# lightec-xyz/bls-verify-gadget

Hardware: AMD Instinct MI355X
Metric: BLS-verify witness instances/sec (full pairing circuit) (higher is better)
Workload: dtype u32 (381-bit Montgomery integers mod the BLS12-381 prime as 12 x 32-bit limbs in memory, products on 14 x 28-bit limbs with 64-bit columns; SHA-256 words)

## Files before the change

__graft_entry__.py:

```python
import importlib
import os
import subprocess
import sys

ROOT = os.path.dirname(os.path.abspath(__file__))
if ROOT not in sys.path:
    sys.path.insert(0, ROOT)


def build():
    pkg = importlib.import_module("bls-verify-gadget_amd")
    pkg.build(force=False)
    subprocess.check_call(["make", "-s", "-C", os.path.join(ROOT, "oracle")])
    subprocess.check_call(["make", "-s", "-C", os.path.join(ROOT, "tests", "hostsim")])
    subprocess.check_call(["make", "-s", "-C", os.path.join(ROOT, "tests", "msg_input")])
    subprocess.check_call(["make", "-s", "-C", os.path.join(ROOT, "tests", "agg_inputs")])
    subprocess.check_call(["make", "-s", "-C", os.path.join(ROOT, "tests", "c_caller")])
    subprocess.check_call(["make", "-s", "-C", os.path.join(ROOT, "tests", "cpp_caller")])
    pkg.lib()
    for s in pkg.EXPORTED_SYMBOLS:
        getattr(pkg.lib(), s)


def smoke():
    import numpy as np
    import torch

    from tests import oracle_lib, synth

    pkg = importlib.import_module("bls-verify-gadget_amd")
    o = oracle_lib.load()
# ... 21 lines not shown
```

bls-verify-gadget_amd/build.py:

```python
import concurrent.futures
import hashlib
import os
import subprocess
import sys

HERE = os.path.dirname(os.path.abspath(__file__))
CSRC = os.path.join(HERE, "csrc")
OUT = os.path.join(HERE, "libblsw.so")
OBJ = os.path.join(HERE, "build_obj")
SOURCES = ["engine.hip", "k_agg_io.hip", "k_bench.hip", "k_cofactor.hip", "k_cofv.hip", "k_g1.hip", "k_g2.hip", "k_map.hip", "k_miller_par.hip", "k_msg.hip", "k_pairing_lane.hip", "k_prepare.hip", "k_r1cs.hip", "k_sha.hip",
           "k_sign.hip", "k_stream.hip", "k_team.hip", "k_values.hip"]
HOST_SOURCES = ["r1cs.cpp"]
HEADERS = sorted(f for f in os.listdir(CSRC) if f.endswith((".hpp", ".h")))
_SHORT_W2 = "the short chains: +4 % on the 20-step job at two waves, neutral in the steady state (profiles/r03_ab_chain_builds.txt)"
CHAIN_UNITS = {
    "k_sha.hip": ("W2", ("inl",), _SHORT_W2),
    "k_g1.hip": ("W2", ("inl",), _SHORT_W2),
    "k_g2.hip": ("OUTLINE", ("inl", "q"), "inlined it takes the whole file and the expansion starves; at two waves it spills 590 registers into its hot loop "
                 "(profiles/r03_ab_chain_builds.txt)"),
    "k_map.hip": ("W2", ("inl", "q"), _SHORT_W2),
    "k_cofactor.hip": ("OUTLINE", ("inl",), "inlined it takes the whole file and the expansion starves; at two waves it spills 2 400 registers into its hot loop "
                       "(profiles/r03_ab_chain_builds.txt)"),
    "k_prepare.hip": ("W2", ("inl", "q"), _SHORT_W2),
    "k_cofv.hip": ("FULL", ("q",), "the serial phases and the join: at two waves the join spills 2 000 registers into its additions"),
}
# ... 136 lines not shown
```

bls-verify-gadget_amd/csrc/chains.hpp:

```cpp
#pragma once
#include "curve.hpp"
#include "tower.hpp"

namespace blsw {

BLSW_HD bool bit_of(const uint32_t* words, int i) { return (words[i >> 5] >> (i & 31)) & 1; }

BLSW_FN bool fp_is_eq_pre_w(Emitter& e, const Fp& diff, const Fp& diff_inv) {
    bool ne = !fp_is_zero(diff);
    e.put_bool(ne);
    e.put(ne ? diff_inv : fp_one());
    return !ne;
}

struct G1ChainOut {
    Fp ax, ay;
};
BLSW_FN Proj<OpsFp> chain_g1_alloc_only(Emitter e_alloc, const Fp& pkx, const Fp& pky) {
    constexpr uint32_t H1[4] = BLSW_H1_WORDS;
    constexpr uint32_t H1INV[8] = BLSW_H1INV_WORDS;
    bool inf = fp_is_zero(pkx) && fp_is_zero(pky);
    Jac1 acc = {pkx, pky, fp_one()};
#pragma unroll 1
    for (int i = BLSW_H1INV_NBITS - 2; i >= 0; i--) {
        acc = jac1_dbl(acc);
        if (bit_of(H1INV, i)) acc = jac1_add_mixed(acc, pkx, pky);
    }
    Fp zi = fp_inv(acc.z);
    Fp zi2 = fp_sqr(zi);
    Fp px = fp_mul(acc.x, zi2), py = fp_mul(acc.y, fp_mul(zi2, zi));
    Proj<OpsFp> ge;
    ge.x = inf ? fp_zero() : px;
    ge.y = inf ? fp_one() : py;
    ge.z = inf ? fp_zero() : fp_one();
    e_alloc.put(ge.x);
    e_alloc.put(ge.y);
    e_alloc.put(ge.z);
    return proj_mul_bits_be_w<OpsFp>(e_alloc, ge, H1, BLSW_H1_NBITS);
}
BLSW_FN G1ChainOut chain_g1_post(Emitter e_notzero, Emitter e_prep, const Proj<OpsFp>& pk) {
    Fp nz = fp_neg(pk.z);
    Fp nzi = fp_inv(nz);
    bool x_eq = fp_is_eq_pre_w(e_notzero, fp_zero(), fp_zero());
    bool y_eq = fp_is_eq_pre_w(e_notzero, nz, nzi);
    bool coords_eq = x_eq && y_eq;
    e_notzero.put_bool(coords_eq);
    bool z_is_zero = fp_is_eq_pre_w(e_notzero, nz, nzi);
    e_notzero.put_bool(!z_is_zero && !coords_eq);
    bool infinity = fp_is_eq_pre_w(e_prep, nz, nzi);
    Fp z_inv = fp_neg(nzi);
    e_prep.put(z_inv);
    Fp nzx = fp_mul_w(e_prep, pk.x, z_inv);
    Fp nzy = fp_mul_w(e_prep, pk.y, z_inv);
// ... 32 lines not shown
    Fp2 l0 = fp2_mul_w(e, ge.x, ge.z);
    Fp2 r0 = fp2_mul_w(e, ge.x, ge.z);
    bool x_eq = fp2_is_eq_w(e, l0, r0);
    Fp2 l1 = fp2_mul_w(e, ge.y, ge.z);
    Fp2 r1 = fp2_mul_w(e, ge.y, ge.z);
    bool y_eq = fp2_is_eq_w(e, l1, r1);
    bool coords_eq = x_eq && y_eq;
    e.put_bool(coords_eq);
    bool za = fp2_is_zero_w(e, ge.z);
    bool zb = fp2_is_zero_w(e, ge.z);
    bool both_zero = za && zb;
    e.put_bool(both_zero);
    e.put_bool(both_zero || coords_eq);
}

BLSW_FN void chain_g2_alloc(Emitter e, const Fp2& sx, const Fp2& sy) {
    constexpr uint32_t RM1[8] = BLSW_RM1_WORDS;
    bool inf = fp2_is_zero(sx) && fp2_is_zero(sy);
    Proj<OpsFp2> ge;
    ge.x = inf ? fp2_zero() : sx;
    ge.y = inf ? fp2_one() : sy;
    ge.z = inf ? fp2_zero() : fp2_one();
    e.put(ge.x.c0);
    e.put(ge.x.c1);
    e.put(ge.y.c0);
    e.put(ge.y.c1);
    e.put(ge.z.c0);
    e.put(ge.z.c1);
    (void)proj_mul_bits_be_w<OpsFp2>(e, ge, RM1, BLSW_RM1_NBITS);
    chain_g2_alloc_tail(e, ge);
}

BLSW_FN Fp2 sswu_pow_c1_w(Emitter& e, const Fp2& v) {
    constexpr uint32_t C1[24] = BLSW_SSWU_C1_WORDS;
    Fp2 r = v;
#pragma unroll 1
    for (int i = BLSW_SSWU_C1_NBITS - 4; i >= 0; i--) {
        r = fp2_sqr_w(e, r);
        if (bit_of(C1, i)) r = fp2_mul_w(e, r, v);
    }
    return r;
}
BLSW_FN bool sswu_sgn0_w(Emitter& e, const Fp2& v) {
    bool sign_0 = fp_to_bits_le_w(e, v.c0);
// ... 381 lines not shown
```

bls-verify-gadget_amd/csrc/curve.hpp:

```cpp
#pragma once
#include "constants.hpp"
#include "gadgets.hpp"

namespace blsw {

struct OpsFp {
    typedef Fp F;
    static BLSW_HD F add(const F& a, const F& b) { return fp_add(a, b); }
    static BLSW_HD F sub(const F& a, const F& b) { return fp_sub(a, b); }
    static BLSW_HD F dbl(const F& a) { return fp_dbl(a); }
    static BLSW_HD F neg(const F& a) { return fp_neg(a); }
    static BLSW_HD F mul_w(Emitter& e, const F& a, const F& b) { return fp_mul_w(e, a, b); }
    static BLSW_HD F sqr_w(Emitter& e, const F& a) { return fp_mul_w(e, a, a); }
    static BLSW_HD F mul3b(const F& a) {
        F a4 = fp_dbl(fp_dbl(a));
        return fp_add(fp_dbl(a4), a4);
    }
    static BLSW_HD F one() { return fp_one(); }
    static BLSW_HD F zero() { return fp_zero(); }
    static BLSW_HD F k3b() { return K_G1_3B(); }
};
struct OpsFp2 {
    typedef Fp2 F;
    static BLSW_HD F add(const F& a, const F& b) { return fp2_add(a, b); }
// ... 70 lines not shown
    F m3 = O::mul_w(e, xx3, bxz3);
    F y = O::add(m2, m3);
    F m4 = O::mul_w(e, yy_p, yz_pairs);
    F m5 = O::mul_w(e, xy_pairs, xx3);
    F z = O::add(m4, m5);
    return {x, y, z};
}
template <class O>
BLSW_FN Proj<O> proj_double_w(Emitter& e, const Proj<O>& p) {
    return proj_double_inl<O>(e, p);
}
template <class O, int ZMODE>
BLSW_FN Proj<O> proj_add_w(Emitter& e, const Proj<O>& a, const Proj<O>& b) {
    return proj_add_inl<O, ZMODE>(e, a, b);
}
template <class O>
BLSW_FN Proj<O> proj_mul_bits_be_w(Emitter& e, const Proj<O>& ge, const uint32_t* words, int nbits) {
    Proj<O> result = ge;
#pragma unroll 1
    for (int i = nbits - 2; i >= 0; i--) {
        result = proj_double_inl<O>(e, result);
        if ((words[i >> 5] >> (i & 31)) & 1) result = proj_add_inl<O, 0>(e, result, ge);
    }
    return result;
}

struct Aff2 {
    Fp2 x, y;
};
BLSW_FN Aff2 nz_double_w(Emitter& e, const Aff2& p) {
    Fp2 x1_sqr = fp2_sqr_w(e, p.x);
    Fp2 num = fp2_add(fp2_dbl(x1_sqr), x1_sqr);
    Fp2 den = fp2_dbl(p.y);
    Fp2 lambda = fp2_div_w(e, num, den);
    Fp2 l2 = fp2_sqr_w(e, lambda);
// ... 95 lines not shown
```

bls-verify-gadget_amd/csrc/engine.hip:

```cpp
#include <cstdio>
#include <cstdlib>
#include <deque>
#include <map>
#include <vector>
#include "kcommon.hpp"
#include "agg_input.hpp"

using namespace blsw;

namespace {

inline int hip_ok(hipError_t e, const char* what) {
    if (e != hipSuccess) {
        fprintf(stderr, "[blsw] %s: %s\n", what, hipGetErrorString(e));
        return BLSW_ERR_HIP;
    }
    return BLSW_OK;
}

struct DeviceGuard {
    int prev = -1;
    bool switched = false;
    explicit DeviceGuard(int dev) {
        if (dev < 0) return;
// ... 101 lines not shown
    }
    if (e->sha) hipStreamDestroy(e->sha);
    if (e->expand) hipStreamDestroy(e->expand);
    if (e->place) hipStreamDestroy(e->place);
    if (e->lat) hipStreamDestroy(e->lat);
    if (e->ev_exp) {
        for (int i = 0; i < 2 * BLSW_MAX_TIMED; i++)
            if (e->ev_exp[i]) hipEventDestroy(e->ev_exp[i]);
        delete[] e->ev_exp;
    }
    for (int i = 0; i < BLSW_MAX_CONSUMED; i++)
        if (e->consumed_ev[i]) hipEventDestroy(e->consumed_ev[i]);
    delete e;
}

static void launch_place(blsw_engine* e, hipStream_t st, const Fp* staging, const Fp* pair, uint32_t split_row, uint64_t first, uint64_t* out, uint64_t out_stride) {
    const uint32_t rows = e->L.n_witness - e->L.sha_bits;
    const unsigned chunks = (rows * 3 + 256 * BLSW_PLACE_ITERS - 1) / (256 * BLSW_PLACE_ITERS);
    dim3 grid2(8 * ((chunks + 7) / 8) * (unsigned)e->n);
    hipLaunchKernelGGL(k_place_field, grid2, dim3(256), 0, st, staging, pair, first, e->L.off_expand, e->L.sha_bits, rows, split_row, out, out_stride, (uint32_t)e->n,
                       e->L.off_sig_alloc, e->modes.g2_team ? e->L.off_pk_not_zero - e->L.off_sig_alloc : 0u, e->LS.off_sig_alloc);
}
static void launch_place_multi(blsw_engine* e, hipStream_t st, const Workspace& ws, const Fp* pair_tiles, uint64_t first_pair, const Fp* inst_tiles, uint64_t first_inst,
                               uint32_t inst_tile_w, const Fp* rows, uint64_t* out, uint64_t out_stride) {
    const blsw_layout_t& L = e->L;
    const blsw_layout_t& S = e->LS;
    const uint32_t K = L.n_pairs, n = (uint32_t)e->n;
    PlaceRuns pr = {};
    pr.n_runs = 6;
    const uint32_t src[7] = {S.off_msg, S.off_pk_alloc, S.off_pk_not_zero, S.off_map0, S.off_prep_h, S.off_prep_pk, ws.rows_p};
    const uint32_t dst[6] = {L.off_msg, L.off_pk_alloc, L.off_pk_not_zero, L.off_map0, L.off_prep_h, L.off_prep_pk};
    const uint32_t str[6] = {L.stride_msg, L.stride_pk_alloc, L.stride_pk_not_zero, L.stride_hash, L.stride_prep_h, L.stride_prep_pk};
    for (int r = 0; r < 7; r++) pr.src_row[r] = src[r];
    for (int r = 0; r < 6; r++) pr.dst_off[r] = dst[r], pr.dst_stride[r] = str[r];
    auto blocks = [](uint32_t rows_, uint32_t n_y) {
        const unsigned chunks = (rows_ * 3 + 256 * BLSW_PLACE_ITERS - 1) / (256 * BLSW_PLACE_ITERS);
// ... 72 lines not shown
    hipEventRecord(b.ev_x[s], e->expand);
    hipStreamWaitEvent(e->place, b.ev_chains, 0);
    hipStreamWaitEvent(e->place, b.ev_x[s], 0);
    if (d.compact) {
        char* dst = reinterpret_cast<char*>(d.compact);
        hipMemcpyAsync(dst + cf.off_staging, ws.staging + (uint64_t)s * (e->n * Kc / 64) * ws.rows_p * 64, cf.staging_bytes, hipMemcpyDeviceToDevice, e->place);
        if (cf.inst_bytes) {
            const uint64_t lane0 = (uint64_t)s * e->n;
            const Fp* src = ws.staging_inst + (lane0 >> 6) * (uint64_t)ws.rows_i * 64 + (lane0 & 63);
            if (cf.inst_tile_w == 64)
                hipMemcpyAsync(dst + cf.off_inst, src, cf.inst_bytes, hipMemcpyDeviceToDevice, e->place);
            else
                hipMemcpy2DAsync(dst + cf.off_inst, e->n * sizeof(Fp), src, 64 * sizeof(Fp), e->n * sizeof(Fp), ws.rows_i, hipMemcpyDeviceToDevice, e->place);
        }
        if (cf.pair_bytes) hipMemcpyAsync(dst + cf.off_pair, ws.pair + (uint64_t)s * e->n * ws.pair_rows, cf.pair_bytes, hipMemcpyDeviceToDevice, e->place);
    }
    if (d.out && e->staged) {
        if (e->L.n_pairs > 1)
            launch_place_multi(e, e->place, ws, ws.staging, (uint64_t)s * e->n * e->L.n_pairs, ws.staging_inst, (uint64_t)s * e->n, 64u,
                               ws.pair + (uint64_t)s * e->n * ws.pair_rows, d.out, d.out_stride);
        else
            launch_place(e, e->place, ws.staging, ws.pair, ws.split_row, (uint64_t)s * e->n, d.out, d.out_stride);
    }
    if (d.out && e->opt.output_form) launch_canonical(e, e->place, d.out, d.out_stride);
    hipEventRecord(b.ev_step[s], e->place);
}
static int pump(blsw_engine* e) {
    while (!e->jobs.empty()) {
        const Job j = e->jobs.front();
        GroupBuf& b = e->buf[j.buf];
        const StepDesc& d = b.h_desc[j.s];
        const void* ptr = tracked_output(e, d);
        int slot = -1;
        if (ptr) {
            slot = consumed_slot(e, ptr);
            if (slot < 0) return BLSW_ERR_ARG;
            if (e->held[slot]) break;
// ... 269 lines not shown
    o->pk_mode = 0;
    o->sig_mode = 0;
    o->msg_mode = 0;
    o->agg_inputs = 0;
    return BLSW_OK;
}

int blsw_engine_workspace_bytes_ex(uint64_t n, uint32_t msg_len, uint32_t max_steps, uint32_t n_buffers, const blsw_engine_options_t* options, uint64_t* bytes) {
    if (!bytes) return BLSW_ERR_ARG;
    if (int rc = check_options(n, msg_len, max_steps, n_buffers, options)) return rc;
    blsw_layout_t L;
    const uint32_t K = options->n_pairs > 1 ? options->n_pairs : 1;
    options_layout(msg_len, options, &L);
    const bool staged = max_steps > 1 || n_buffers > 1;
    uint64_t need = 0;
    const Modes all[3] = {{true, false}, {true, true}, {false, false}};
    const uint64_t small_steps = BLSW_LATENCY_MAX_LANES / (n * K) < max_steps ? BLSW_LATENCY_MAX_LANES / (n * K) : max_steps;
    for (const Modes& m : all) {
        uint64_t t = carve(nullptr, n * max_steps * K, L, staged, m, n * max_steps).total_bytes;
        need = t > need ? t : need;
        if (small_steps) {
            t = carve(nullptr, n * small_steps * K, L, staged, m, n * small_steps).total_bytes;
            need = t > need ? t : need;
        }
    }
    if (K > 1) need = align_up(need, 256) + miller_par_bytes(n * max_steps, K);
    *bytes = (uint64_t)n_buffers * align_up(need, 4096);
    return BLSW_OK;
}
int blsw_engine_workspace_bytes(uint64_t n, uint32_t msg_len, uint32_t max_steps, uint32_t n_buffers, uint64_t* bytes) {
    blsw_engine_options_t o;
// ... 23 lines not shown
        if (hipFuncGetAttributes(&fa, reinterpret_cast<const void*>(k_pairing)) == hipSuccess && fa.localSizeBytes) stack = fa.localSizeBytes;
        const uint64_t projected = stack * 64ull * (uint64_t)cus * 32ull * n_buffers;
        if (projected > (16ull << 30)) {
            fprintf(stderr, "[blsw] pairing_mode 1 with %u group buffers needs about %.1f GB of per-queue scratch: refused (use pairing_mode 0 or n_buffers <= 3)\n",
                    n_buffers, projected / 1e9);
            return BLSW_ERR_SCRATCH;
        }
    }
    blsw_engine* e = new blsw_engine();
    e->n = n;
    e->msg_len = msg_len;
    e->max_steps = max_steps;
    e->opt = *options;
    e->opt.device = dev;
    e->device = dev;
    e->modes = {options->pairing_mode == 0, options->g2_mode == 1};
    e->staged = max_steps > 1 || n_buffers > 1;
    e->cofactor_mode = options->cofactor_mode;
    e->chains_inlined = options->chain_variant == 2 || (options->chain_variant == 0 && !e->staged);
    options_layout(msg_len, options, &e->L);
    e->LS = e->L.n_pairs > 1 ? staging_layout_multi(e->L).LS : staging_layout(e->L, e->modes);
    for (int i = 0; i < BLSW_MAX_CONSUMED; i++) {
        e->consumed_ptr[i] = nullptr;
        e->consumed_ev[i] = nullptr;
        e->consumed_live[i] = false;
        e->held[i] = false;
        e->refs[i] = 0;
    }
    e->nbuf = (int)n_buffers;
    int rc = BLSW_OK;
    auto chk = [&](hipError_t err, const char* what) {
        if (rc == BLSW_OK && hip_ok(err, what)) rc = BLSW_ERR_HIP;
        return rc == BLSW_OK;
    };
    e->ev_exp = new hipEvent_t[2 * BLSW_MAX_TIMED]();
// ... 171 lines not shown
}
int blsw_engine_expand_compact(blsw_engine_t* e, const void* d_compact, uint64_t* d_witness, uint64_t witness_stride, void* stream_) {
    if (!e || !e->staged || !compact_shape_ok(e->n, e->L.n_pairs) || !d_compact || !d_witness || witness_stride < e->L.n_witness) return BLSW_ERR_ARG;
    DeviceGuard guard(e->device);
    hipStream_t st = reinterpret_cast<hipStream_t>(stream_);
    const uint32_t K = e->L.n_pairs;
    const Workspace w = carve(nullptr, e->n * K, e->L, true, e->modes, e->n);
    const CompactForm cf = compact_form(e->n, w, K);
    const char* src = reinterpret_cast<const char*>(d_compact);
    ExpandArgs xa = {reinterpret_cast<const uint32_t*>(src), w.sha_words, 0, e->L.sha_bits, e->L.off_expand, d_witness, witness_stride, K, K > 1 ? e->L.stride_hash : 0u, 0, (int)e->opt.output_form};
    engine_expand(e, st, xa, (unsigned)(e->n * K));
    if (K > 1)
        launch_place_multi(e, st, w, reinterpret_cast<const Fp*>(src + cf.off_staging), 0, reinterpret_cast<const Fp*>(src + cf.off_inst), 0, cf.inst_tile_w,
                           reinterpret_cast<const Fp*>(src + cf.off_pair), d_witness, witness_stride);
    else
        launch_place(e, st, reinterpret_cast<const Fp*>(src + cf.off_staging), reinterpret_cast<const Fp*>(src + cf.off_pair), w.split_row, 0, d_witness, witness_stride);
    if (e->opt.output_form) launch_canonical(e, st, d_witness, witness_stride);
    return hip_ok(hipGetLastError(), "expand compact");
}

int blsw_engine_flush(blsw_engine_t* e, void* stream_) {
    if (!e) return BLSW_ERR_ARG;
    DeviceGuard guard(e->device);
    hipStream_t st = reinterpret_cast<hipStream_t>(stream_);
    int rc = launch_group(e);
    e->ramp_pos = 0;
    if (rc) return rc;
    if ((rc = pump(e))) return rc;
    for (int k = 0; k < e->nbuf; k++)
        if (e->buf[k].used && e->buf[k].jobs_left == 0) hipStreamWaitEvent(st, e->buf[k].ev_done, 0);
    return hip_ok(hipGetLastError(), "flush");
// ... 382 lines not shown
```

bls-verify-gadget_amd/csrc/k_g1.hip:

```cpp
#include "kcommon.hpp"
#include "agg_input.hpp"

namespace blsw {

__global__ __launch_bounds__(64) BLSW_CHAIN_ATTR void BLSW_K(k_g1)(Group g) {
    if (g.chain_prio) __builtin_amdgcn_s_setprio(3);
    uint64_t I = (uint64_t)blockIdx.x * blockDim.x + threadIdx.x;
    const bool params = g.L.params_mode && I >= g.N;
    if (params) I -= g.N;
    if (I >= g.N) return;
    LaneId id = lane_id(g, I);
    const Fp* p = reinterpret_cast<const Fp*>(g.desc[id.s].pk + (uint64_t)id.f * 12);
    Emitter e_alloc = EMITJ(g, id, off_pk_alloc, stride_pk_alloc), e_nz = EMITJ(g, id, off_pk_not_zero, stride_pk_not_zero),
            e_prep = EMITJ(g, id, off_prep_pk, stride_prep_pk);
    Fp x = ld_fp(p), y = ld_fp(p + 1);
    if (params) {
        e_alloc = EMIT(g, id, off_params_alloc);
        e_prep = EMIT(g, id, off_prep_g1);
        e_nz.base = nullptr;
        x = K_G1_GEN_X();
        y = fp_neg(K_G1_GEN_NEG_Y());
    }
    Proj<OpsFp> pk;
    if (g.L.pk_mode && !params) {
        const bool inf = fp_is_zero(x) && fp_is_zero(y);
        pk = {inf ? fp_zero() : x, inf ? fp_one() : y, inf ? fp_zero() : fp_one()};
        const uint32_t k0 = g.L.n_instance_vars - 3 - (g.L.sig_mode ? 6 : 0);
        put_instance(g, id, k0, pk.x);
        put_instance(g, id, k0 + 1, pk.y);
        put_instance(g, id, k0 + 2, pk.z);
    } else {
        pk = chain_g1_alloc_only(e_alloc, x, y);
    }
    if (!params) put_instance(g, id, 0, fp_one());
    if (params) pk.y = fp_neg(pk.y);
    G1ChainOut o = chain_g1_post(e_nz, e_prep, pk);
    if (params) return;
    st_fp(g.ws.pkaff + I, o.ax);
    st_fp(g.ws.pkaff + g.N + I, o.ay);
}

__global__ __launch_bounds__(64) BLSW_CHAIN_ATTR void BLSW_K(k_agg_keys)(Group g, Fp* keyproj) {
    if (g.chain_prio) __builtin_amdgcn_s_setprio(3);
    uint64_t t = (uint64_t)blockIdx.x * blockDim.x + threadIdx.x;
    const uint64_t N = g.N, nk = g.L.n_keys;
    if (t >= N * nk) return;
    uint32_t k = (uint32_t)(t / N);
// ... 53 lines not shown
```

bls-verify-gadget_amd/csrc/k_g2.hip:

```cpp
#include "kcommon.hpp"

namespace blsw {

__global__ __launch_bounds__(64) BLSW_CHAIN_ATTR void BLSW_K(k_g2_alloc)(Group g) {
    if (g.chain_prio) __builtin_amdgcn_s_setprio(3);
    const uint64_t I = item_index();
    if (I >= g.N) return;
    LaneId id = lane_id(g, I);
    const Fp* p = reinterpret_cast<const Fp*>(g.desc[id.s].sig + (uint64_t)id.i * 24);
    Fp2 sx = {ld_fp(p), ld_fp(p + 1)}, sy = {ld_fp(p + 2), ld_fp(p + 3)};
    chain_g2_alloc(EMIT(g, id, off_sig_alloc), sx, sy);
}

}
```

bls-verify-gadget_amd/csrc/kcommon.hpp:

```cpp
#pragma once
#include <hip/hip_runtime.h>
#include <stdio.h>
#include <stdlib.h>
#include <string.h>
#define BLSW_ATTR_W2 __attribute__((amdgpu_waves_per_eu(2, 2)))
#if defined(BLSW_KVARIANT_QUAD)
#define BLSW_QUAD 1
#define BLSW_INLINE_CHAINS 1
#define BLSW_CHAIN_ATTR
#define BLSW_K(name) name##_q
#define BLSW_LPI 4u
#elif defined(BLSW_KVARIANT_INL)
#define BLSW_INLINE_CHAINS 1
#define BLSW_CHAIN_ATTR
#define BLSW_K(name) name##_inl
#define BLSW_LPI 1u
#else
#if defined(BLSW_CHAIN_W2) || defined(BLSW_CHAIN_FULL)
#define BLSW_INLINE_CHAINS 1
#endif
#ifdef BLSW_CHAIN_W2
#define BLSW_CHAIN_ATTR BLSW_ATTR_W2
#else
#define BLSW_CHAIN_ATTR
#endif
#define BLSW_K(name) name
#define BLSW_LPI 1u
#endif
#include "chains.hpp"
#include "cofactor_vf.hpp"
#include "prepare_vf.hpp"
#include "layout.h"

namespace blsw {

__device__ __forceinline__ uint64_t item_index() { return ((uint64_t)blockIdx.x * blockDim.x + threadIdx.x) / BLSW_LPI; }
__device__ __forceinline__ bool item_leader() { return BLSW_LPI == 1u || (threadIdx.x & (BLSW_LPI - 1u)) == 0u; }
inline unsigned item_grid(uint64_t items, unsigned lpi) { return (unsigned)((items * lpi + 63) / 64); }

struct Workspace {
    uint32_t* bits;
    Fp* u;
    Fp* q;
    Fp* h;
    Fp* pkaff;
    Fp* coeff_h;
    Fp* coeff_sig;
    uint64_t n_sig;
    Fp* keyproj;
    Fp* staging;
    Fp* staging_inst;
    uint32_t rows_p, rows_i;
    uint64_t staging_rows;
    Fp* pair;
    uint32_t split_row;
    uint32_t pair_rows;
    uint64_t sha_words;
    Fp* cofv;
    Fp* prepv_h;
    Fp* prepv_sig;
    uint64_t total_bytes;
};
#define BLSW_LATENCY_MAX_LANES 8192
inline uint64_t align_up(uint64_t x, uint64_t a) { return (x + a - 1) / a * a; }
BLSW_HD uint64_t bits_tile_words(uint64_t sha_words) { return sha_words * 64; }
struct Modes {
    bool pairing_team;
    bool g2_team;
};
constexpr Modes DEFAULT_MODES = {true, false};
inline blsw_layout_t staging_layout(const blsw_layout_t& L, const Modes& m) {
    blsw_layout_t S = L;
    uint32_t* f = &S.off_msg;
    const uint32_t* g = &L.off_msg;
    for (int k = 0; k < 15; k++) f[k] = g[k] > L.off_expand ? g[k] - L.sha_bits : g[k];
    if (L.off_prep_g1 > L.off_expand) S.off_prep_g1 = L.off_prep_g1 - L.sha_bits;
    if (m.g2_team) {
        const uint32_t lo = L.off_sig_alloc, len = L.off_pk_not_zero - L.off_sig_alloc;
        for (int k = 0; k < 15; k++)
            if (f[k] > lo) f[k] -= len;
        if (S.off_prep_g1 > lo) S.off_prep_g1 -= len;
        S.off_sig_alloc = L.n_witness - L.sha_bits - len;
    }
    return S;
}
struct MultiStaging {
    blsw_layout_t LS;
    uint32_t rows_p, rows_i, split, pair_rows;
};
inline MultiStaging staging_layout_multi(const blsw_layout_t& L) {
    MultiStaging m;
    m.LS = L;
    blsw_layout_t& S = m.LS;
    uint32_t o = 0;
    S.off_msg = o;
    o += L.stride_msg;
    S.off_pk_alloc = o;
// ... 33 lines not shown
        return reinterpret_cast<char*>(base) + o;
    };
    w.bits = reinterpret_cast<uint32_t*>(take(bits_tile_words(w.sha_words) * (align_up(N, 64) / 64) * 4));
    w.u = reinterpret_cast<Fp*>(take(4 * N * sizeof(Fp)));
    w.q = reinterpret_cast<Fp*>(take(12 * N * sizeof(Fp)));
    w.h = reinterpret_cast<Fp*>(take(6 * N * sizeof(Fp)));
    w.pkaff = reinterpret_cast<Fp*>(take(2 * N * sizeof(Fp)));
    w.coeff_h = reinterpret_cast<Fp*>(take(272ull * N * sizeof(Fp)));
    w.coeff_sig = reinterpret_cast<Fp*>(take(272ull * n_sig * sizeof(Fp)));
    w.n_sig = n_sig;
    w.keyproj = L.n_keys && !L.pk_mode ? reinterpret_cast<Fp*>(take(3ull * N * L.n_keys * sizeof(Fp))) : nullptr;
    const bool small = N <= BLSW_LATENCY_MAX_LANES;
    w.cofv = small ? reinterpret_cast<Fp*>(take((uint64_t)BLSW_COFV_ELEMS * N * sizeof(Fp))) : nullptr;
    w.prepv_h = small ? reinterpret_cast<Fp*>(take((uint64_t)BLSW_PREPV_ELEMS * N * sizeof(Fp))) : nullptr;
    w.prepv_sig = small ? reinterpret_cast<Fp*>(take((uint64_t)BLSW_PREPV_ELEMS * n_sig * sizeof(Fp))) : nullptr;
    w.staging_rows = L.n_witness - L.sha_bits;
    if (L.n_pairs > 1 && with_staging) {
        const MultiStaging ms = staging_layout_multi(L);
        w.rows_p = ms.rows_p;
        w.rows_i = ms.rows_i;
        w.split_row = ms.split;
        w.pair_rows = ms.pair_rows;
        w.staging = reinterpret_cast<Fp*>(take((uint64_t)w.rows_p * align_up(N, 64) * sizeof(Fp)));
        w.staging_inst = reinterpret_cast<Fp*>(take((uint64_t)w.rows_i * align_up(n_sig, 64) * sizeof(Fp)));
        w.pair = reinterpret_cast<Fp*>(take((uint64_t)w.pair_rows * n_sig * sizeof(Fp)));
        w.total_bytes = off;
        return w;
    }
    w.split_row = m.pairing_team ? staging_layout(L, m).off_miller : (uint32_t)w.staging_rows;
    w.pair_rows = (uint32_t)w.staging_rows - w.split_row;
    w.rows_p = w.rows_i = w.split_row;
    w.staging = with_staging ? reinterpret_cast<Fp*>(take((uint64_t)w.split_row * align_up(N, 64) * sizeof(Fp))) : nullptr;
    w.staging_inst = w.staging;
    w.pair = with_staging && w.pair_rows ? reinterpret_cast<Fp*>(take((uint64_t)w.pair_rows * N * sizeof(Fp))) : nullptr;
    w.total_bytes = off;
    return w;
}

struct StepDesc {
    const uint64_t* pk;
    const uint64_t* sig;
    const uint8_t* msg;
    uint64_t* out;
    uint64_t out_stride;
    int32_t* result;
    const uint64_t* keys;
    const uint8_t* bitmap;
    uint32_t* count;
    void* compact;
    const int32_t* status;
    uint64_t* inst;
};
__device__ __forceinline__ int32_t step_result(const StepDesc& d, uint32_t i, bool res) {
    if (d.status && (d.status[2 * i] | d.status[2 * i + 1])) return 0;
    return res ? 1 : 0;
}
struct CompactForm {
    uint64_t bits_bytes, staging_bytes, inst_bytes, pair_bytes, off_staging, off_inst, off_pair, total;
    uint32_t inst_tile_w;
};
inline CompactForm compact_form(uint64_t n, const Workspace& w, uint32_t K = 1) {
    CompactForm c;
    c.bits_bytes = bits_tile_words(w.sha_words) * (n * K / 64) * 4;
    c.staging_bytes = (uint64_t)w.rows_p * n * K * sizeof(Fp);
    c.inst_bytes = K > 1 ? (uint64_t)w.rows_i * n * sizeof(Fp) : 0;
    c.inst_tile_w = n % 64 == 0 ? 64u : (uint32_t)n;
    c.pair_bytes = (uint64_t)w.pair_rows * n * sizeof(Fp);
    c.off_staging = align_up(c.bits_bytes, 256);
    c.off_inst = align_up(c.off_staging + c.staging_bytes, 256);
    c.off_pair = align_up(c.off_inst + c.inst_bytes, 256);
    c.total = align_up(c.off_pair + c.pair_bytes, 256);
    return c;
}
inline bool compact_shape_ok(uint64_t n, uint32_t K) { return K <= 1 ? n % 64 == 0 : ((n * K) % 64 == 0 && (n % 64 == 0 || 64 % n == 0)); }
struct Group {
    uint64_t N;
    uint32_t n;
    uint32_t K;
    uint32_t msg_len;
    uint32_t msg_wit_len;
    const StepDesc* desc;
    blsw_layout_t L;
    blsw_layout_t LS;
    Workspace ws;
    int chain_prio;
    int canonical;
// ... 48 lines not shown
        const uint32_t rows = per_pair ? g.ws.rows_p : g.ws.rows_i;
        e.base = reinterpret_cast<uint32_t*>(tiles + (id.I >> 6) * (uint64_t)rows * 64 + (id.I & 63));
        e.pos = off_staging;
        e.stride = 64 * 12;
        return e;
    }
    const StepDesc& d = g.desc[id.s];
    e.base = d.out ? reinterpret_cast<uint32_t*>(d.out + (uint64_t)id.i * d.out_stride * 6) : nullptr;
    e.pos = off_full;
    e.stride = 12;
    return e;
}
#define EMIT(g, id, field) emitter(g, id, (g).L.field, (g).LS.field, false)
#define EMITJ(g, id, field, stride) emitter(g, id, (g).L.field + (id).j * (g).L.stride, (g).LS.field + (id).j * (g).LS.stride, true)

__device__ __forceinline__ Proj<OpsFp2> ld_proj2(const Fp* p, uint64_t n) {
    Proj<OpsFp2> r;
    r.x = ld_fp2(p, n);
    r.y = ld_fp2(p + 2 * n, n);
    r.z = ld_fp2(p + 4 * n, n);
    return r;
}

struct CoeffStrided {
    Fp* p;
    uint64_t n;
    __device__ __forceinline__ void st(uint32_t idx, const Fp& v) const {
        if (item_leader()) st_fp(p + (uint64_t)idx * n, v);
    }
    __device__ __forceinline__ Fp ld(uint32_t idx) const { return ld_fp(p + (uint64_t)idx * n); }
// ... 40 lines not shown
BLSW_CHAIN_Q(k_cofv_bwd, (Group g, int s))
BLSW_CHAIN_Q(k_cofv_acc, (Group g, int s))
BLSW_CHAIN_Q(k_cofv_az, (Group g))
__global__ void k_cofv_aff(Group g, uint32_t lo, uint32_t cnt);
__global__ void k_cofv_dbl_w(Group g);
__global__ void k_cofv_add_w(Group g);
__global__ void k_cofv_join(Group g);
__global__ void k_sha_values(Group g);
__global__ void k_msg_input(Group g);
__global__ void k_agg_instance(Group g, uint32_t n_elems, uint32_t s0);
__global__ void k_map_values(Group g);
__global__ void k_cofactor_values(Group g);
__global__ void k_place_field(const Fp* __restrict__ staging, const Fp* __restrict__ pair, uint64_t first, uint32_t off_expand, uint32_t sha_bits,
                              uint32_t staging_rows, uint32_t split_row, uint64_t* __restrict__ d_witness, uint64_t stride, uint32_t n_inst, uint32_t moved_lo,
                              uint32_t moved_len, uint32_t moved_at);
__global__ void k_canonical_rows(uint64_t* __restrict__ d_witness, uint64_t stride, uint32_t off_expand, uint32_t sha_bits, uint32_t rows, uint32_t K, uint32_t stride_hash);
__global__ void k_digest(const uint64_t* __restrict__ w, uint64_t stride, uint64_t n_words, uint64_t* __restrict__ digest);
__global__ void k_pairing(Group g);
__global__ void k_pairing_team(Group g);
__global__ void k_pairing_team_pv(Group g);
__global__ void k_g2_alloc_team(Group g);
__global__ void k_pairing_team_multi(Group gs, uint32_t K, uint64_t n_h);
__global__ void k_decode(const uint8_t* __restrict__ pk48, const uint8_t* __restrict__ sig96, uint64_t n, uint64_t* pk_xy, uint64_t* sig_xy, int32_t* status);
__global__ void k_h_to_affine(uint64_t n, Workspace ws, uint64_t* d_out);
__global__ void k_decode_points(uint32_t group, const uint8_t* __restrict__ in, uint64_t m, Fp* xy, int32_t* st);
__global__ void k_sum_points(uint32_t group, const Fp* __restrict__ xy, const int32_t* __restrict__ pst, uint32_t k, uint64_t n, uint8_t* out, int32_t* status);
__global__ void k_sign(uint64_t n, Workspace ws, const uint8_t* __restrict__ sk32, uint8_t* sig96, uint64_t* sig_xy, uint8_t* pk48, uint64_t* pk_xy, int32_t* status);
__global__ void k_bench_mad(uint32_t iters, uint32_t* out);
__global__ void k_bench_fill(uint4* __restrict__ dst, uint64_t n16);
__global__ void k_bench_fpmul(uint32_t iters, uint32_t* out);
// ... 170 lines not shown
```

include/blsw.h:

```cpp
#ifndef BLSW_H
#define BLSW_H
#include <stdint.h>
#ifdef __cplusplus
extern "C" {
#endif

#define BLSW_ABI_VERSION 13

#define BLSW_OK 0
#define BLSW_ERR_ARG 1
#define BLSW_ERR_WORKSPACE 2
#define BLSW_ERR_HIP 3
#define BLSW_ERR_NO_DEVICE 4
#define BLSW_ERR_SCRATCH 5
#define BLSW_ERR_BUSY 6

#define BLSW_ST_OK 0
#define BLSW_ST_BAD_ENCODING 1
#define BLSW_ST_NOT_ON_CURVE 2
#define BLSW_ST_NOT_IN_SUBGROUP 3
#define BLSW_ST_IDENTITY 4
#define BLSW_ST_INVALID_SECRET_KEY 5

typedef struct {
// ... 152 lines not shown
```

Measured before the change: 128,300.

## Checkpoint scalar-mul accumulators and re-emit G1/G2 allocation witnesses at placement

During the G1 and G2 cofactor-multiplication chains, the code now stores only the running projective accumulator per iteration into a compact checkpoint tile and stops writing the full allocation witness rows into staging. At placement, new kernels rebuild each iteration's double/add witnesses from the checkpoints in parallel (one grid row per iteration) and write them straight to the output, with a constexpr plan giving each iteration's row offset. The aim is to shrink staging traffic and the copy of allocation rows, in exchange for recomputing doubles and adds in the placement phase and adding checkpoint memory and two extra launches. It is enabled only for staged runs without g2_team, msg_input, keys or multi-pair modes.

```diff
diff --git a/__graft_entry__.py b/__graft_entry__.py
--- a/__graft_entry__.py
+++ b/__graft_entry__.py
@@ -15,6 +15,7 @@
     subprocess.check_call(["make", "-s", "-C", os.path.join(ROOT, "tests", "hostsim")])
     subprocess.check_call(["make", "-s", "-C", os.path.join(ROOT, "tests", "msg_input")])
     subprocess.check_call(["make", "-s", "-C", os.path.join(ROOT, "tests", "agg_inputs")])
+    subprocess.check_call(["make", "-s", "-C", os.path.join(ROOT, "tests", "emit_host")])
     subprocess.check_call(["make", "-s", "-C", os.path.join(ROOT, "tests", "c_caller")])
     subprocess.check_call(["make", "-s", "-C", os.path.join(ROOT, "tests", "cpp_caller")])
     pkg.lib()
diff --git a/bls-verify-gadget_amd/build.py b/bls-verify-gadget_amd/build.py
--- a/bls-verify-gadget_amd/build.py
+++ b/bls-verify-gadget_amd/build.py
@@ -8,7 +8,7 @@
 CSRC = os.path.join(HERE, "csrc")
 OUT = os.path.join(HERE, "libblsw.so")
 OBJ = os.path.join(HERE, "build_obj")
-SOURCES = ["engine.hip", "k_agg_io.hip", "k_bench.hip", "k_cofactor.hip", "k_cofv.hip", "k_g1.hip", "k_g2.hip", "k_map.hip", "k_miller_par.hip", "k_msg.hip", "k_pairing_lane.hip", "k_prepare.hip", "k_r1cs.hip", "k_sha.hip",
+SOURCES = ["engine.hip", "k_agg_io.hip", "k_bench.hip", "k_cofactor.hip", "k_cofv.hip", "k_emit.hip", "k_g1.hip", "k_g2.hip", "k_map.hip", "k_miller_par.hip", "k_msg.hip", "k_pairing_lane.hip", "k_prepare.hip", "k_r1cs.hip", "k_sha.hip",
            "k_sign.hip", "k_stream.hip", "k_team.hip", "k_values.hip"]
 HOST_SOURCES = ["r1cs.cpp"]
 HEADERS = sorted(f for f in os.listdir(CSRC) if f.endswith((".hpp", ".h")))
diff --git a/bls-verify-gadget_amd/csrc/chains.hpp b/bls-verify-gadget_amd/csrc/chains.hpp
--- a/bls-verify-gadget_amd/csrc/chains.hpp
+++ b/bls-verify-gadget_amd/csrc/chains.hpp
@@ -16,7 +16,8 @@
 struct G1ChainOut {
     Fp ax, ay;
 };
-BLSW_FN Proj<OpsFp> chain_g1_alloc_only(Emitter e_alloc, const Fp& pkx, const Fp& pky) {
+template <class S = NoCkpt>
+BLSW_FN Proj<OpsFp> chain_g1_alloc_only(Emitter e_alloc, const Fp& pkx, const Fp& pky, const S& sink = S()) {
     constexpr uint32_t H1[4] = BLSW_H1_WORDS;
     constexpr uint32_t H1INV[8] = BLSW_H1INV_WORDS;
     bool inf = fp_is_zero(pkx) && fp_is_zero(pky);
@@ -36,7 +37,7 @@
     e_alloc.put(ge.x);
     e_alloc.put(ge.y);
     e_alloc.put(ge.z);
-    return proj_mul_bits_be_w<OpsFp>(e_alloc, ge, H1, BLSW_H1_NBITS);
+    return proj_mul_bits_be_w<OpsFp, S>(e_alloc, ge, H1, BLSW_H1_NBITS, sink);
 }
 BLSW_FN G1ChainOut chain_g1_post(Emitter e_notzero, Emitter e_prep, const Proj<OpsFp>& pk) {
     Fp nz = fp_neg(pk.z);
@@ -99,7 +100,8 @@
     e.put_bool(both_zero || coords_eq);
 }
 
-BLSW_FN void chain_g2_alloc(Emitter e, const Fp2& sx, const Fp2& sy) {
+template <class S = NoCkpt>
+BLSW_FN void chain_g2_alloc(Emitter e, const Fp2& sx, const Fp2& sy, const S& sink = S()) {
     constexpr uint32_t RM1[8] = BLSW_RM1_WORDS;
     bool inf = fp2_is_zero(sx) && fp2_is_zero(sy);
     Proj<OpsFp2> ge;
@@ -112,7 +114,7 @@
     e.put(ge.y.c1);
     e.put(ge.z.c0);
     e.put(ge.z.c1);
-    (void)proj_mul_bits_be_w<OpsFp2>(e, ge, RM1, BLSW_RM1_NBITS);
+    (void)proj_mul_bits_be_w<OpsFp2, S>(e, ge, RM1, BLSW_RM1_NBITS, sink);
     chain_g2_alloc_tail(e, ge);
 }
 
diff --git a/bls-verify-gadget_amd/csrc/curve.hpp b/bls-verify-gadget_amd/csrc/curve.hpp
--- a/bls-verify-gadget_amd/csrc/curve.hpp
+++ b/bls-verify-gadget_amd/csrc/curve.hpp
@@ -108,11 +108,16 @@
 BLSW_FN Proj<O> proj_add_w(Emitter& e, const Proj<O>& a, const Proj<O>& b) {
     return proj_add_inl<O, ZMODE>(e, a, b);
 }
-template <class O>
-BLSW_FN Proj<O> proj_mul_bits_be_w(Emitter& e, const Proj<O>& ge, const uint32_t* words, int nbits) {
+struct NoCkpt {
+    template <class P>
+    BLSW_HD void put(uint32_t, const P&) const {}
+};
+template <class O, class S = NoCkpt>
+BLSW_FN Proj<O> proj_mul_bits_be_w(Emitter& e, const Proj<O>& ge, const uint32_t* words, int nbits, const S& sink = S()) {
     Proj<O> result = ge;
 #pragma unroll 1
     for (int i = nbits - 2; i >= 0; i--) {
+        sink.put((uint32_t)(nbits - 2 - i), result);
         result = proj_double_inl<O>(e, result);
         if ((words[i >> 5] >> (i & 31)) & 1) result = proj_add_inl<O, 0>(e, result, ge);
     }
diff --git a/bls-verify-gadget_amd/csrc/emit_alloc.hpp b/bls-verify-gadget_amd/csrc/emit_alloc.hpp
--- /dev/null
+++ b/bls-verify-gadget_amd/csrc/emit_alloc.hpp
@@ -0,0 +1,128 @@
+#pragma once
+#include "chains.hpp"
+#include "layout.h"
+
+namespace blsw {
+
+#define BLSW_EMIT_G1_ITERS (BLSW_H1_NBITS - 1)
+#define BLSW_EMIT_G2_ITERS (BLSW_RM1_NBITS - 1)
+#define BLSW_EMIT_G2_ROW0 (3u * BLSW_EMIT_G1_ITERS)
+#define BLSW_EMIT_CKPT_ROWS (BLSW_EMIT_G2_ROW0 + 6u * BLSW_EMIT_G2_ITERS)
+#define BLSW_EMIT_ITEMS (BLSW_EMIT_G1_ITERS + BLSW_EMIT_G2_ITERS + 1)
+#define BLSW_EMIT_ROWS ((uint32_t)SEG_PK_ALLOC + (uint32_t)SEG_SIG_ALLOC)
+
+struct EmitPlan {
+    uint16_t pos_g1[BLSW_EMIT_G1_ITERS];
+    uint16_t pos_g2[BLSW_EMIT_G2_ITERS];
+    uint16_t g1_adds, g2_adds;
+    uint16_t g1_end, g2_tail, g2_end;
+};
+constexpr bool emit_bit(const uint32_t* words, int i) { return (words[i >> 5] >> (i & 31)) & 1; }
+constexpr EmitPlan emit_plan() {
+    constexpr uint32_t H1[4] = BLSW_H1_WORDS;
+    constexpr uint32_t RM1[8] = BLSW_RM1_WORDS;
+    EmitPlan p = {};
+    uint32_t pos = 3;
+    for (int k = 0; k < BLSW_EMIT_G1_ITERS; k++) {
+        p.pos_g1[k] = (uint16_t)pos;
+        pos += 11;
+        if (emit_bit(H1, BLSW_H1_NBITS - 2 - k)) pos += 12, p.g1_adds++;
+    }
+    p.g1_end = (uint16_t)pos;
+    pos = 6;
+    for (int k = 0; k < BLSW_EMIT_G2_ITERS; k++) {
+        p.pos_g2[k] = (uint16_t)pos;
+        pos += 30;
+        if (emit_bit(RM1, BLSW_RM1_NBITS - 2 - k)) pos += 36, p.g2_adds++;
+    }
+    p.g2_tail = (uint16_t)pos;
+    p.g2_end = (uint16_t)(pos + 35);
+    return p;
+}
+static_assert(emit_plan().g1_end == SEG_PK_ALLOC && emit_plan().g1_adds == 47, "G1 allocation: the plan must count what chain_g1_alloc_only emits");
+static_assert(emit_plan().g2_end == SEG_SIG_ALLOC && emit_plan().g2_adds == 132, "G2 allocation: the plan must count what chain_g2_alloc emits");
+constexpr bool emit_top_bits_set() {
+    constexpr uint32_t H1[4] = BLSW_H1_WORDS;
+    constexpr uint32_t RM1[8] = BLSW_RM1_WORDS;
+    return emit_bit(H1, BLSW_H1_NBITS - 1) && emit_bit(RM1, BLSW_RM1_NBITS - 1);
+}
+static_assert(emit_top_bits_set(), "the scalars' top bits are set: the first addition is the constant-zero special case, iteration 0 starts from ge");
+static_assert(SEG_SIG_ALLOC < 65536, "EmitPlan holds positions as uint16_t");
+
+template <class C>
+struct CkptSinkG1 {
+    C c;
+    BLSW_HD void put(uint32_t k, const Proj<OpsFp>& r) const {
+        c.st(3 * k, r.x);
+        c.st(3 * k + 1, r.y);
+        c.st(3 * k + 2, r.z);
+    }
+};
+template <class C>
+struct CkptSinkG2 {
+    C c;
+    BLSW_HD void put(uint32_t k, const Proj<OpsFp2>& r) const {
+        const uint32_t row = BLSW_EMIT_G2_ROW0 + 6 * k;
+        c.st(row, r.x.c0);
+        c.st(row + 1, r.x.c1);
+        c.st(row + 2, r.y.c0);
+        c.st(row + 3, r.y.c1);
+        c.st(row + 4, r.z.c0);
+        c.st(row + 5, r.z.c1);
+    }
+};
+template <class C>
+BLSW_HD Proj<OpsFp> ckpt_ld_g1(const C& c, uint32_t k) {
+    return {c.ld(3 * k), c.ld(3 * k + 1), c.ld(3 * k + 2)};
+}
+template <class C>
+BLSW_HD Proj<OpsFp2> ckpt_ld_g2(const C& c, uint32_t k) {
+    const uint32_t row = BLSW_EMIT_G2_ROW0 + 6 * k;
+    return {{c.ld(row), c.ld(row + 1)}, {c.ld(row + 2), c.ld(row + 3)}, {c.ld(row + 4), c.ld(row + 5)}};
+}
+
+template <class O>
+BLSW_HD void emit_mul_iter(Emitter e, const Proj<O>& result, const Proj<O>& ge, bool add) {
+    const Proj<O> d = proj_double_inl<O>(e, result);
+    if (add) (void)proj_add_inl<O, 0>(e, d, ge);
+}
+template <class C>
+BLSW_HD void emit_alloc_iter(uint32_t it, const C& ck, Emitter e_pk, Emitter e_sig) {
+    constexpr uint32_t H1[4] = BLSW_H1_WORDS;
+    constexpr uint32_t RM1[8] = BLSW_RM1_WORDS;
+    constexpr EmitPlan plan = emit_plan();
+    if (it < BLSW_EMIT_G1_ITERS) {
+        e_pk.pos += plan.pos_g1[it];
+        emit_mul_iter<OpsFp>(e_pk, ckpt_ld_g1(ck, it), ckpt_ld_g1(ck, 0), bit_of(H1, BLSW_H1_NBITS - 2 - (int)it));
+    } else {
+        const uint32_t k = it - BLSW_EMIT_G1_ITERS;
+        e_sig.pos += plan.pos_g2[k];
+        emit_mul_iter<OpsFp2>(e_sig, ckpt_ld_g2(ck, k), ckpt_ld_g2(ck, 0), bit_of(RM1, BLSW_RM1_NBITS - 2 - (int)k));
+    }
+}
+template <class C>
+BLSW_HD void emit_alloc_ends(const C& ck, Emitter e_pk, Emitter e_sig) {
+    constexpr EmitPlan plan = emit_plan();
+    const Proj<OpsFp> pk = ckpt_ld_g1(ck, 0);
+    e_pk.put(pk.x);
+    e_pk.put(pk.y);
+    e_pk.put(pk.z);
+    const Proj<OpsFp2> ge = ckpt_ld_g2(ck, 0);
+    e_sig.put(ge.x.c0);
+    e_sig.put(ge.x.c1);
+    e_sig.put(ge.y.c0);
+    e_sig.put(ge.y.c1);
+    e_sig.put(ge.z.c0);
+    e_sig.put(ge.z.c1);
+    e_sig.pos += plan.g2_tail - 6u;
+    chain_g2_alloc_tail(e_sig, ge);
+}
+template <class C>
+BLSW_HD void emit_alloc_item(uint32_t it, const C& ck, Emitter e_pk, Emitter e_sig) {
+    if (it < BLSW_EMIT_ITEMS - 1)
+        emit_alloc_iter(it, ck, e_pk, e_sig);
+    else
+        emit_alloc_ends(ck, e_pk, e_sig);
+}
+
+}
diff --git a/bls-verify-gadget_amd/csrc/engine.hip b/bls-verify-gadget_amd/csrc/engine.hip
--- a/bls-verify-gadget_amd/csrc/engine.hip
+++ b/bls-verify-gadget_amd/csrc/engine.hip
@@ -139,12 +139,23 @@
     delete e;
 }
 
-static void launch_place(blsw_engine* e, hipStream_t st, const Fp* staging, const Fp* pair, uint32_t split_row, uint64_t first, uint64_t* out, uint64_t out_stride) {
-    const uint32_t rows = e->L.n_witness - e->L.sha_bits;
+static void launch_place(blsw_engine* e, hipStream_t st, const Fp* staging, const Fp* pair, const Fp* ckpt, uint32_t split_row, uint64_t first, uint64_t* out,
+                         uint64_t out_stride) {
+    const bool emit = e->modes.emit_alloc;
+    const uint32_t rows = e->L.n_witness - e->L.sha_bits - (emit ? BLSW_EMIT_ROWS : 0u);
     const unsigned chunks = (rows * 3 + 256 * BLSW_PLACE_ITERS - 1) / (256 * BLSW_PLACE_ITERS);
     dim3 grid2(8 * ((chunks + 7) / 8) * (unsigned)e->n);
+    uint32_t moved_lo = e->L.off_sig_alloc, moved_len = e->modes.g2_team ? e->L.off_pk_not_zero - e->L.off_sig_alloc : 0u, moved_at = e->LS.off_sig_alloc;
+    if (emit) moved_lo = e->L.off_pk_alloc, moved_len = BLSW_EMIT_ROWS, moved_at = 0xffffffffu;
     hipLaunchKernelGGL(k_place_field, grid2, dim3(256), 0, st, staging, pair, first, e->L.off_expand, e->L.sha_bits, rows, split_row, out, out_stride, (uint32_t)e->n,
-                       e->L.off_sig_alloc, e->modes.g2_team ? e->L.off_pk_not_zero - e->L.off_sig_alloc : 0u, e->LS.off_sig_alloc);
+                       moved_lo, moved_len, moved_at);
+    if (emit) {
+        const unsigned gx = (unsigned)((e->n + 63) / 64);
+        const uint32_t ckpt_rows = BLSW_EMIT_CKPT_ROWS;
+        hipLaunchKernelGGL(k_emit_alloc_ends, dim3(gx), dim3(64), 0, st, ckpt, first, ckpt_rows, e->L.off_pk_alloc, e->L.off_sig_alloc, out, out_stride, (uint32_t)e->n);
+        hipLaunchKernelGGL(k_emit_alloc, dim3(gx, BLSW_EMIT_ITEMS - 1), dim3(64), 0, st, ckpt, first, ckpt_rows, e->L.off_pk_alloc, e->L.off_sig_alloc, out, out_stride,
+                           (uint32_t)e->n);
+    }
 }
 static void launch_place_multi(blsw_engine* e, hipStream_t st, const Workspace& ws, const Fp* pair_tiles, uint64_t first_pair, const Fp* inst_tiles, uint64_t first_inst,
                                uint32_t inst_tile_w, const Fp* rows, uint64_t* out, uint64_t out_stride) {
@@ -247,13 +258,14 @@
                 hipMemcpy2DAsync(dst + cf.off_inst, e->n * sizeof(Fp), src, 64 * sizeof(Fp), e->n * sizeof(Fp), ws.rows_i, hipMemcpyDeviceToDevice, e->place);
         }
         if (cf.pair_bytes) hipMemcpyAsync(dst + cf.off_pair, ws.pair + (uint64_t)s * e->n * ws.pair_rows, cf.pair_bytes, hipMemcpyDeviceToDevice, e->place);
+        if (cf.ckpt_bytes) hipMemcpyAsync(dst + cf.off_ckpt, ws.ckpt + (uint64_t)s * (e->n / 64) * ws.ckpt_rows * 64, cf.ckpt_bytes, hipMemcpyDeviceToDevice, e->place);
     }
     if (d.out && e->staged) {
         if (e->L.n_pairs > 1)
             launch_place_multi(e, e->place, ws, ws.staging, (uint64_t)s * e->n * e->L.n_pairs, ws.staging_inst, (uint64_t)s * e->n, 64u,
                                ws.pair + (uint64_t)s * e->n * ws.pair_rows, d.out, d.out_stride);
         else
-            launch_place(e, e->place, ws.staging, ws.pair, ws.split_row, (uint64_t)s * e->n, d.out, d.out_stride);
+            launch_place(e, e->place, ws.staging, ws.pair, ws.ckpt, ws.split_row, (uint64_t)s * e->n, d.out, d.out_stride);
     }
     if (d.out && e->opt.output_form) launch_canonical(e, e->place, d.out, d.out_stride);
     hipEventRecord(b.ev_step[s], e->place);
@@ -553,7 +565,7 @@
     options_layout(msg_len, options, &L);
     const bool staged = max_steps > 1 || n_buffers > 1;
     uint64_t need = 0;
-    const Modes all[3] = {{true, false}, {true, true}, {false, false}};
+    const Modes all[3] = {{true, false, false}, {true, true, false}, {false, false, false}};
     const uint64_t small_steps = BLSW_LATENCY_MAX_LANES / (n * K) < max_steps ? BLSW_LATENCY_MAX_LANES / (n * K) : max_steps;
     for (const Modes& m : all) {
         uint64_t t = carve(nullptr, n * max_steps * K, L, staged, m, n * max_steps).total_bytes;
@@ -607,11 +619,12 @@
     e->opt = *options;
     e->opt.device = dev;
     e->device = dev;
-    e->modes = {options->pairing_mode == 0, options->g2_mode == 1};
     e->staged = max_steps > 1 || n_buffers > 1;
     e->cofactor_mode = options->cofactor_mode;
     e->chains_inlined = options->chain_variant == 2 || (options->chain_variant == 0 && !e->staged);
     options_layout(msg_len, options, &e->L);
+    e->modes = {options->pairing_mode == 0, options->g2_mode == 1, false};
+    e->modes.emit_alloc = emit_alloc_ok(e->L, e->staged, e->modes.g2_team, options_msg_input(options));
     e->LS = e->L.n_pairs > 1 ? staging_layout_multi(e->L).LS : staging_layout(e->L, e->modes);
     for (int i = 0; i < BLSW_MAX_CONSUMED; i++) {
         e->consumed_ptr[i] = nullptr;
@@ -813,7 +826,8 @@
         launch_place_multi(e, st, w, reinterpret_cast<const Fp*>(src + cf.off_staging), 0, reinterpret_cast<const Fp*>(src + cf.off_inst), 0, cf.inst_tile_w,
                            reinterpret_cast<const Fp*>(src + cf.off_pair), d_witness, witness_stride);
     else
-        launch_place(e, st, reinterpret_cast<const Fp*>(src + cf.off_staging), reinterpret_cast<const Fp*>(src + cf.off_pair), w.split_row, 0, d_witness, witness_stride);
+        launch_place(e, st, reinterpret_cast<const Fp*>(src + cf.off_staging), reinterpret_cast<const Fp*>(src + cf.off_pair), reinterpret_cast<const Fp*>(src + cf.off_ckpt),
+                     w.split_row, 0, d_witness, witness_stride);
     if (e->opt.output_form) launch_canonical(e, st, d_witness, witness_stride);
     return hip_ok(hipGetLastError(), "expand compact");
 }
diff --git a/bls-verify-gadget_amd/csrc/k_emit.hip b/bls-verify-gadget_amd/csrc/k_emit.hip
--- /dev/null
+++ b/bls-verify-gadget_amd/csrc/k_emit.hip
@@ -0,0 +1,32 @@
+#include "kcommon.hpp"
+
+namespace blsw {
+
+struct EmitLane {
+    CkptTile ck;
+    Emitter e_pk, e_sig;
+};
+__device__ __forceinline__ EmitLane emit_lane(const Fp* ckpt, uint64_t lane, uint32_t ckpt_rows, uint32_t off_pk_alloc, uint32_t off_sig_alloc, uint64_t* vec) {
+    EmitLane l;
+    l.ck = ckpt_tile(const_cast<Fp*>(ckpt), ckpt_rows, lane);
+    l.e_pk.base = l.e_sig.base = reinterpret_cast<uint32_t*>(vec);
+    l.e_pk.pos = off_pk_alloc;
+    l.e_sig.pos = off_sig_alloc;
+    return l;
+}
+__global__ __launch_bounds__(64) void k_emit_alloc(const Fp* __restrict__ ckpt, uint64_t first, uint32_t ckpt_rows, uint32_t off_pk_alloc, uint32_t off_sig_alloc,
+                                                   uint64_t* __restrict__ d_witness, uint64_t stride, uint32_t n_inst) {
+    const uint32_t inst = blockIdx.x * 64 + threadIdx.x;
+    if (inst >= n_inst) return;
+    const EmitLane l = emit_lane(ckpt, first + inst, ckpt_rows, off_pk_alloc, off_sig_alloc, d_witness + (uint64_t)inst * stride * 6);
+    emit_alloc_iter(blockIdx.y, l.ck, l.e_pk, l.e_sig);
+}
+__global__ __launch_bounds__(64) void k_emit_alloc_ends(const Fp* __restrict__ ckpt, uint64_t first, uint32_t ckpt_rows, uint32_t off_pk_alloc, uint32_t off_sig_alloc,
+                                                        uint64_t* __restrict__ d_witness, uint64_t stride, uint32_t n_inst) {
+    const uint32_t inst = blockIdx.x * 64 + threadIdx.x;
+    if (inst >= n_inst) return;
+    const EmitLane l = emit_lane(ckpt, first + inst, ckpt_rows, off_pk_alloc, off_sig_alloc, d_witness + (uint64_t)inst * stride * 6);
+    emit_alloc_ends(l.ck, l.e_pk, l.e_sig);
+}
+
+}
diff --git a/bls-verify-gadget_amd/csrc/k_g1.hip b/bls-verify-gadget_amd/csrc/k_g1.hip
--- a/bls-verify-gadget_amd/csrc/k_g1.hip
+++ b/bls-verify-gadget_amd/csrc/k_g1.hip
@@ -30,7 +30,9 @@
         put_instance(g, id, k0 + 1, pk.y);
         put_instance(g, id, k0 + 2, pk.z);
     } else {
-        pk = chain_g1_alloc_only(e_alloc, x, y);
+        const CkptSinkG1<CkptTile> sink = {ckpt_tile(g.ws.ckpt, g.ws.ckpt_rows, I)};
+        if (sink.c.p) e_alloc.base = nullptr;
+        pk = chain_g1_alloc_only(e_alloc, x, y, sink);
     }
     if (!params) put_instance(g, id, 0, fp_one());
     if (params) pk.y = fp_neg(pk.y);
diff --git a/bls-verify-gadget_amd/csrc/k_g2.hip b/bls-verify-gadget_amd/csrc/k_g2.hip
--- a/bls-verify-gadget_amd/csrc/k_g2.hip
+++ b/bls-verify-gadget_amd/csrc/k_g2.hip
@@ -9,7 +9,10 @@
     LaneId id = lane_id(g, I);
     const Fp* p = reinterpret_cast<const Fp*>(g.desc[id.s].sig + (uint64_t)id.i * 24);
     Fp2 sx = {ld_fp(p), ld_fp(p + 1)}, sy = {ld_fp(p + 2), ld_fp(p + 3)};
-    chain_g2_alloc(EMIT(g, id, off_sig_alloc), sx, sy);
+    Emitter e = EMIT(g, id, off_sig_alloc);
+    const CkptSinkG2<CkptTile> sink = {ckpt_tile(g.ws.ckpt, g.ws.ckpt_rows, I)};
+    if (sink.c.p) e.base = nullptr;
+    chain_g2_alloc(e, sx, sy, sink);
 }
 
 }
diff --git a/bls-verify-gadget_amd/csrc/kcommon.hpp b/bls-verify-gadget_amd/csrc/kcommon.hpp
--- a/bls-verify-gadget_amd/csrc/kcommon.hpp
+++ b/bls-verify-gadget_amd/csrc/kcommon.hpp
@@ -31,6 +31,7 @@
 #include "cofactor_vf.hpp"
 #include "prepare_vf.hpp"
 #include "layout.h"
+#include "emit_alloc.hpp"
 
 namespace blsw {
 
@@ -59,6 +60,8 @@
     Fp* cofv;
     Fp* prepv_h;
     Fp* prepv_sig;
+    Fp* ckpt;
+    uint32_t ckpt_rows;
     uint64_t total_bytes;
 };
 #define BLSW_LATENCY_MAX_LANES 8192
@@ -67,8 +70,12 @@
 struct Modes {
     bool pairing_team;
     bool g2_team;
-};
-constexpr Modes DEFAULT_MODES = {true, false};
+    bool emit_alloc;
+};
+constexpr Modes DEFAULT_MODES = {true, false, false};
+inline bool emit_alloc_ok(const blsw_layout_t& L, bool staged, bool g2_team, bool msg_input) {
+    return staged && !g2_team && !msg_input && !L.n_keys && L.n_pairs <= 1 && !L.pk_mode && !L.sig_mode && !L.params_mode;
+}
 inline blsw_layout_t staging_layout(const blsw_layout_t& L, const Modes& m) {
     blsw_layout_t S = L;
     uint32_t* f = &S.off_msg;
@@ -81,6 +88,12 @@
             if (f[k] > lo) f[k] -= len;
         if (S.off_prep_g1 > lo) S.off_prep_g1 -= len;
         S.off_sig_alloc = L.n_witness - L.sha_bits - len;
+    }
+    if (m.emit_alloc) {
+        const uint32_t lo = L.off_pk_alloc;
+        for (int k = 0; k < 15; k++)
+            if (f[k] > lo) f[k] -= BLSW_EMIT_ROWS;
+        S.off_pk_alloc = S.off_sig_alloc = 0xffffffffu;
     }
     return S;
 }
@@ -144,7 +157,9 @@
     w.cofv = small ? reinterpret_cast<Fp*>(take((uint64_t)BLSW_COFV_ELEMS * N * sizeof(Fp))) : nullptr;
     w.prepv_h = small ? reinterpret_cast<Fp*>(take((uint64_t)BLSW_PREPV_ELEMS * N * sizeof(Fp))) : nullptr;
     w.prepv_sig = small ? reinterpret_cast<Fp*>(take((uint64_t)BLSW_PREPV_ELEMS * n_sig * sizeof(Fp))) : nullptr;
-    w.staging_rows = L.n_witness - L.sha_bits;
+    w.staging_rows = L.n_witness - L.sha_bits - (m.emit_alloc ? BLSW_EMIT_ROWS : 0u);
+    w.ckpt = nullptr;
+    w.ckpt_rows = 0;
     if (L.n_pairs > 1 && with_staging) {
         const MultiStaging ms = staging_layout_multi(L);
         w.rows_p = ms.rows_p;
@@ -163,6 +178,10 @@
     w.staging = with_staging ? reinterpret_cast<Fp*>(take((uint64_t)w.split_row * align_up(N, 64) * sizeof(Fp))) : nullptr;
     w.staging_inst = w.staging;
     w.pair = with_staging && w.pair_rows ? reinterpret_cast<Fp*>(take((uint64_t)w.pair_rows * N * sizeof(Fp))) : nullptr;
+    if (m.emit_alloc && with_staging) {
+        w.ckpt_rows = BLSW_EMIT_CKPT_ROWS;
+        w.ckpt = reinterpret_cast<Fp*>(take((uint64_t)w.ckpt_rows * align_up(N, 64) * sizeof(Fp)));
+    }
     w.total_bytes = off;
     return w;
 }
@@ -186,7 +205,7 @@
     return res ? 1 : 0;
 }
 struct CompactForm {
-    uint64_t bits_bytes, staging_bytes, inst_bytes, pair_bytes, off_staging, off_inst, off_pair, total;
+    uint64_t bits_bytes, staging_bytes, inst_bytes, pair_bytes, ckpt_bytes, off_staging, off_inst, off_pair, off_ckpt, total;
     uint32_t inst_tile_w;
 };
 inline CompactForm compact_form(uint64_t n, const Workspace& w, uint32_t K = 1) {
@@ -199,7 +218,9 @@
     c.off_staging = align_up(c.bits_bytes, 256);
     c.off_inst = align_up(c.off_staging + c.staging_bytes, 256);
     c.off_pair = align_up(c.off_inst + c.inst_bytes, 256);
-    c.total = align_up(c.off_pair + c.pair_bytes, 256);
+    c.ckpt_bytes = (uint64_t)w.ckpt_rows * n * sizeof(Fp);
+    c.off_ckpt = align_up(c.off_pair + c.pair_bytes, 256);
+    c.total = align_up(c.off_ckpt + c.ckpt_bytes, 256);
     return c;
 }
 inline bool compact_shape_ok(uint64_t n, uint32_t K) { return K <= 1 ? n % 64 == 0 : ((n * K) % 64 == 0 && (n % 64 == 0 || 64 % n == 0)); }
@@ -278,6 +299,16 @@
 #define EMIT(g, id, field) emitter(g, id, (g).L.field, (g).LS.field, false)
 #define EMITJ(g, id, field, stride) emitter(g, id, (g).L.field + (id).j * (g).L.stride, (g).LS.field + (id).j * (g).LS.stride, true)
 
+struct CkptTile {
+    Fp* p;
+    __device__ __forceinline__ void st(uint32_t row, const Fp& v) const {
+        if (p && item_leader()) st_fp(p + (uint64_t)row * 64, v);
+    }
+    __device__ __forceinline__ Fp ld(uint32_t row) const { return ld_fp(p + (uint64_t)row * 64); }
+};
+__device__ __forceinline__ CkptTile ckpt_tile(Fp* ckpt, uint32_t ckpt_rows, uint64_t I) {
+    return {ckpt ? ckpt + (I >> 6) * (uint64_t)ckpt_rows * 64 + (I & 63) : nullptr};
+}
 __device__ __forceinline__ Proj<OpsFp2> ld_proj2(const Fp* p, uint64_t n) {
     Proj<OpsFp2> r;
     r.x = ld_fp2(p, n);
@@ -348,6 +379,10 @@
 __global__ void k_place_field(const Fp* __restrict__ staging, const Fp* __restrict__ pair, uint64_t first, uint32_t off_expand, uint32_t sha_bits,
                               uint32_t staging_rows, uint32_t split_row, uint64_t* __restrict__ d_witness, uint64_t stride, uint32_t n_inst, uint32_t moved_lo,
                               uint32_t moved_len, uint32_t moved_at);
+__global__ void k_emit_alloc(const Fp* __restrict__ ckpt, uint64_t first, uint32_t ckpt_rows, uint32_t off_pk_alloc, uint32_t off_sig_alloc, uint64_t* __restrict__ d_witness,
+                             uint64_t stride, uint32_t n_inst);
+__global__ void k_emit_alloc_ends(const Fp* __restrict__ ckpt, uint64_t first, uint32_t ckpt_rows, uint32_t off_pk_alloc, uint32_t off_sig_alloc, uint64_t* __restrict__ d_witness,
+                                  uint64_t stride, uint32_t n_inst);
 __global__ void k_canonical_rows(uint64_t* __restrict__ d_witness, uint64_t stride, uint32_t off_expand, uint32_t sha_bits, uint32_t rows, uint32_t K, uint32_t stride_hash);
 __global__ void k_digest(const uint64_t* __restrict__ w, uint64_t stride, uint64_t n_words, uint64_t* __restrict__ digest);
 __global__ void k_pairing(Group g);
diff --git a/include/blsw.h b/include/blsw.h
--- a/include/blsw.h
+++ b/include/blsw.h
@@ -5,7 +5,7 @@
 extern "C" {
 #endif
 
-#define BLSW_ABI_VERSION 13
+#define BLSW_ABI_VERSION 14
 
 #define BLSW_OK 0
 #define BLSW_ERR_ARG 1
```

Measured after the change: 121,600. 0.948x the previous value.
